# klae01/ddim-audio

Hardware: AMD Instinct MI355X
Metric: DDIM denoising steps/sec (U-Net fwd/s), 1000-step sample, spectrogram batch (higher is better)
Workload: dtype bf16; 1 GPU; BASELINE configs[1]: batch 8/GPU x [2,1024,256] spectrograms, audio.yml U-Net (47.2M params, hash-filled weights; FNet GEMM operands bf16), generalized_steps eta=0 over the 1000-step schedule, one hipGraph per step (inside the forward two batch shards on two streams, fork mask 0x1003f); global_batch=8, t_size=1024, parallelism=batch-sharded x1, no collective in the loop

## Files before the change

### ddim_audio_amd/csrc/api.cpp

```cpp
#include "../../include/ddimx.h"

#include <stdarg.h>
#include <math.h>
#include <stdio.h>
#include <stdlib.h>
#include <string.h>

#include <functional>
#include <string>
#include <vector>

#include "conv_mfma.h"
#include "kernels.h"
#include "train_kernels.h"
#include "wgrad_mfma.h"
#include "conv_pipe.h"

namespace ddimx {
struct Knobs {
    int fnet_dense, conv_pipe, pipe_tpw, bwd_stats_fused, gn_dbg, conv_wreg, conv_wps, conv_var, wgrad_split, wgrad_side, wgrad_hold;
    Knobs() {
        auto geti = [](const char* name, int dflt) { const char* e = getenv(name); return e ? atoi(e) : dflt; };
        conv_var = geti("DDIMX_CONV_VAR", -1);
        conv_wps = geti("DDIMX_CONV_WPS", 0);
// ... 315 lines not shown

static size_t conv_stats_floats(int dtype, int mode, int cin, int cout, int B, int Hv, int Wv) {
    size_t mx = 0;
    for (int var = 0; var < 8; ++var) {
        ConvGeom g;
        if (conv_geometry(dtype, mode, cin, cout, var, &g) != hipSuccess) continue;
        const size_t n = (size_t)B * cdiv(Wv, g.tw) * cdiv(Hv, g.th) * g.classes * g.nout * 2;
        if (n > mx) mx = n;
    }
    if (mode == CONV3 && cin == cout && dtype == DT_BF16) {
        WregGeom wg;
        if (wreg_geometry(CONV3, cin, cout, &wg) == hipSuccess) {
            const size_t n = (size_t)B * cdiv(Wv, wg.tw) * cdiv(Hv, wg.th) * cout * 2;
            if (n > mx) mx = n;
        }
        PipeGeom pg;
        if (pipe_geometry(cin, &pg) == hipSuccess) {
            const size_t n = (size_t)B * cdiv(Wv, pg.tw) * cdiv(Hv, pg.th) * kGnSlab;
            if (n > mx) mx = n;
        }
    }
    if (mode != CONV3 && dtype == DT_BF16) {
        WregGeom wg;
        const int nout = mode == UP4 ? 2 * cout : cout, ncls = mode == UP4 ? 2 : 1;
        if (wreg_geometry(mode, cin, nout, &wg) == hipSuccess) {
            const size_t n = (size_t)B * cdiv(Wv, wg.tw) * cdiv(Hv, wg.th) * ncls * nout * 2;
            if (n > mx) mx = n;
        }
    }
    return mx;
}

static void carve(const ddimx_ctx* c, char* base, int B, int T, Ws* w) {
    const ddimx_config& f = c->cfg;
    const int L = c->L;
    const size_t es = esz(c->dtype);
    Carver cv{base, 0};
    w->temb_h1 = (float*)cv.take((size_t)B * 512 * 4);
    w->temb_h2 = (float*)cv.take((size_t)B * 512 * 4);
    w->temb = (float*)cv.take((size_t)B * c->E * 4);
    const size_t lvl0 = (size_t)B * T * f.f_size * f.ch[0] * es;
    w->A = cv.take(lvl0);
    w->xd.resize(L); w->xu.resize(L);
    size_t stats_f = (size_t)B * conv_in_nparts(T, f.f_size) * (f.ch[0] * 2 > kGnSlab ? f.ch[0] * 2 : kGnSlab);
    size_t hmax = 0;
    int cmax = 0;
    for (int l = 0; l < L; ++l) {
        const int H = T >> l, W = f.f_size >> l, C = f.ch[l];
        const size_t bytes = (size_t)B * H * W * C * es;
        w->xd[l] = cv.take(bytes);
        w->xu[l] = cv.take(bytes);
        if (bytes > hmax) hmax = bytes;
        if (C > cmax) cmax = C;
        size_t s = conv_stats_floats(c->dtype, CONV3, C, C, B, H, W);
        if (s > stats_f) stats_f = s;
        s = (size_t)B * resid_nparts(c->dtype, H * W, C) * (C * 2 > kGnSlab ? C * 2 : kGnSlab);
        if (s > stats_f) stats_f = s;
        if (l > 0) {
            s = conv_stats_floats(c->dtype, DOWN4, f.ch[l - 1], C, B, H, W);
            if (s > stats_f) stats_f = s;
            s = conv_stats_floats(c->dtype, UP4, C, f.ch[l - 1], B, H, W);
            if (s > stats_f) stats_f = s;
        }
    }
    w->h1 = cv.take(hmax);
    w->h2 = cv.take(hmax);
    w->stats_per_sample = stats_f / B;
    w->h_per_sample = hmax / B;
    w->cmax = cmax;
    w->stats = (float*)cv.take(stats_f * 4);
    w->stats2 = (float*)cv.take(stats_f * 4);
    w->scale = (float*)cv.take((size_t)B * cmax * 4);
    w->shift = (float*)cv.take((size_t)B * cmax * 4);
    const int S = T >> (L - 1);
    const size_t M = (size_t)B * S;
    const int hid = f.fnet_hidden, inter = f.fnet_inter;
    w->ln0 = (float*)cv.take((size_t)B * (S > 32 ? S : 32) * c->width * 4);
    w->X = (float*)cv.take(M * hid * 4);
    w->Ut = (float*)cv.take((size_t)B * 2 * hid * S * 4);
    w->Z = (float*)cv.take(M * hid * 4);
    w->Y = (float*)cv.take(M * hid * 4);
    w->Hb = (float*)cv.take(M * inter * 4);
    w->O = (float*)cv.take(M * c->width * 4);
    w->pz = (float*)cv.take((size_t)B * (hid / 16) * 64 * 4);
    w->pv = (float*)cv.take((size_t)B * (hid / 32) * 64 * 4);
    w->zc = (float*)cv.take((size_t)B * 32 * hid * 4);
    w->hc = (float*)cv.take((size_t)B * 32 * inter * 4);
    w->vc = (float*)cv.take((size_t)B * 32 * hid * 4);
    {
        const int bf = c->fnet_bf16;
        const int shp[6][5] = {{(int)M, hid, c->width, 1, bf}, {2 * hid, S, hid, B, 0}, {S, hid, S, B, 0},
                               {(int)M, inter, hid, 1, bf}, {(int)M, hid, inter, 1, bf}, {(int)M, c->width, hid, 1, bf}};
        size_t mx = 0;
        for (auto& q : shp) {
            const size_t n = (size_t)kMaxSplitK * q[3] * q[0] * q[1];
            if (n > mx) mx = n;
        }
        w->gpart_per_sample = mx / B;
        w->gpart = (float*)cv.take(mx * 4);
    }
    w->total = cv.off;
}

struct ConvCall {
    int dtype, mode, cin, cout;
    const void* in; const void* w; const float* bias; const float* chan_add; int chan_add_stride;
    const float* in_scale; const float* in_shift; int xf; int act;
    const void* skip; void* out; float* stats;
    int B, Hin, Win;
    unsigned long long* stamps = nullptr;
    bool batch_plan = false;
    const void* aux = nullptr; const float* aux_scale = nullptr; const float* aux_shift = nullptr; int bwd_mode = 0;
    GnIn gn = {};
    bool groups = false;
    const void* wf = nullptr;
    int kernel_pref = 0;
};

static thread_local bool g_batch_plan = false;
struct BatchPlanScope {
    BatchPlanScope() { g_batch_plan = true; }
    ~BatchPlanScope() { g_batch_plan = false; }
};
struct ConvPlan { ConvGeom g; int var, Hv, Wv, tiles_x, tiles_y, tiles_per_wg, wgs_per_sample; bool wreg, pipe; };
static bool pipe_eligible(const ConvCall& q, PipeGeom* pg) {
    if (q.kernel_pref == 1 || !((knobs().conv_pipe >> (q.cin == 32 ? 0 : 1)) & 1 || q.kernel_pref == 2)) return false;
    if (!q.wf || q.dtype != DT_BF16 || q.mode != CONV3 || q.cin != q.cout || q.act != 1 || q.aux || q.bwd_mode || q.skip || q.batch_plan || g_batch_plan)
        return false;
    if (q.xf != XF_AFFINE && q.xf != XF_AFFINE_SILU) return false;
    if (q.stats && !q.groups) return false;
    if (pipe_geometry(q.cin, pg) != hipSuccess) return false;
    return q.Hin % pg->th == 0 && q.Win % pg->tw == 0;
}
static bool wreg_eligible(const ConvCall& q, WregGeom* wg) {
    if (!knobs().conv_wreg || !q.wf || q.dtype != DT_BF16 || q.act > 1 || q.aux || q.bwd_mode || q.batch_plan || g_batch_plan) return false;
    if (q.skip && q.mode != UP4) return false;
    if (q.xf != XF_NONE && q.xf != XF_AFFINE && q.xf != XF_AFFINE_SILU) return false;
    if (wreg_geometry(q.mode, q.cin, q.mode == UP4 ? 2 * q.cout : q.cout, wg) != hipSuccess) return false;
    const int sxy = q.mode == DOWN4 ? 2 : 1;
    return q.Hin % (wg->th * sxy) == 0 && q.Win % (wg->tw * sxy) == 0;
}
static int conv_plan(const ConvCall& q, ConvPlan* p) {
    ConvGeom& g = p->g;
    p->wreg = false;
    p->pipe = false;
    PipeGeom pgm;
    if (pipe_eligible(q, &pgm)) {
        p->pipe = true;
        p->Hv = q.Hin; p->Wv = q.Win; p->var = 0;
        g.th = pgm.th; g.tw = pgm.tw; g.nb = g.nout = q.cout; g.classes = 1; g.lds_bytes = pgm.lds_bytes; g.nthreads = pgm.nthreads;
        p->tiles_x = q.Win / pgm.tw;
        p->tiles_y = q.Hin / pgm.th;
        const int tiles_s = p->tiles_x * p->tiles_y;
        int tpw = 8;
        if (const int v = knobs().pipe_tpw; v > 0) tpw = q.cin == 32 ? (v & 0xff) : ((v >> 8) ? (v >> 8) : tpw);
        if (tpw > tiles_s) tpw = tiles_s;
        p->tiles_per_wg = tpw;
        p->wgs_per_sample = cdiv(tiles_s, tpw);
        return 0;
    }
    if (q.kernel_pref == 2) return fail("conv %d->%d %dx%d xf=%d act=%d: not eligible for the software-pipelined kernel", q.cin, q.cout, q.Hin, q.Win, q.xf, q.act);
    WregGeom wgm;
    if (wreg_eligible(q, &wgm)) {
        p->wreg = true;
        const int sxy = q.mode == DOWN4 ? 2 : 1;
        p->Hv = q.Hin / sxy; p->Wv = q.Win / sxy; p->var = 0;
        g.th = wgm.th; g.tw = wgm.tw; g.nout = q.mode == UP4 ? 2 * q.cout : q.cout; g.nb = g.nout / wgm.nsplit; g.classes = q.mode == UP4 ? 2 : 1;
        g.lds_bytes = wgm.lds_bytes; g.nthreads = wgm.nthreads;
        p->tiles_x = p->Wv / wgm.tw;
        p->tiles_y = p->Hv / wgm.th;
        const int tiles_s = p->tiles_x * p->tiles_y;
        int wps = tiles_s < 128 ? tiles_s : 128;
        if (tiles_s / 4 > wps) wps = tiles_s / 4;
        if (const int v = knobs().conv_wps; v > 0) wps = v < tiles_s ? v : tiles_s;
        if (q.mode == CONV3 && q.cin == 96 && tiles_s >= 4 && wps > tiles_s / 2) wps = tiles_s / 2;
        if (q.mode != CONV3 && tiles_s >= 64 && cdiv(tiles_s, wps) < 2) wps = tiles_s / 2;
        p->tiles_per_wg = cdiv(tiles_s, wps);
        p->wgs_per_sample = cdiv(tiles_s, p->tiles_per_wg);
        return 0;
    }
    if (q.mode == DOWN4 && ((q.Hin | q.Win) & 1)) return fail("downsample needs even H, W (got %d x %d)", q.Hin, q.Win);
    p->Hv = q.mode == DOWN4 ? q.Hin / 2 : q.Hin;
    p->Wv = q.mode == DOWN4 ? q.Win / 2 : q.Win;
    p->var = conv_pick_variant(q.dtype, q.mode, q.cin, q.cout, (q.batch_plan || g_batch_plan) ? q.B : 0, p->Hv, p->Wv);
    if (conv_geometry(q.dtype, q.mode, q.cin, q.cout, p->var, &g) != hipSuccess)
        return fail("conv %d->%d mode %d dtype %d: no kernel", q.cin, q.cout, q.mode, q.dtype);
    p->tiles_x = cdiv(p->Wv, g.tw);
    p->tiles_y = cdiv(p->Hv, g.th);
    const int tiles_s = p->tiles_x * p->tiles_y;
    int wps = tiles_s < 128 ? tiles_s : 128;
    if (tiles_s / 4 > wps) wps = tiles_s / 4;
    if (q.cin >= 64 && tiles_s >= 512 && wps < 256) wps = 256;
    if (q.mode != CONV3 && tiles_s == 128) wps = 64;
    if (const int v = knobs().conv_wps; v > 0) wps = v < tiles_s ? v : tiles_s;
    p->tiles_per_wg = cdiv(tiles_s, wps);
    p->wgs_per_sample = cdiv(tiles_s, p->tiles_per_wg);
    return 0;
}
constexpr int kNumCUs = 256;
constexpr int kGnFuseConvRounds = 3, kGnFuseResidRounds = 2;
static int conv_rounds(const ConvPlan& p, int B) {
    const long long wgs = (long long)p.wgs_per_sample * B * (p.g.nout / p.g.nb) * p.g.classes;
    int per_cu = (160 * 1024) / p.g.lds_bytes;
    if (per_cu < 1) per_cu = 1;
    if (per_cu > 2048 / p.g.nthreads) per_cu = 2048 / p.g.nthreads;
    return (int)((wgs + (long long)kNumCUs * per_cu - 1) / ((long long)kNumCUs * per_cu));
}
static int run_conv(const ConvCall& q, hipStream_t s, int* nparts, int* Cs) {
    ConvPlan pl;
    CHK(conv_plan(q, &pl));
    const ConvGeom& g = pl.g;
    if (pl.wreg || pl.pipe) {
        WregArgs f;
        memset(&f, 0, sizeof(f));
        f.in = q.in; f.wf = q.wf; f.skip = q.skip; f.bias = q.bias; f.chan_add = q.chan_add; f.chan_add_stride = q.chan_add_stride;
        f.in_scale = q.in_scale; f.in_shift = q.in_shift; f.gn = q.gn; f.out = q.out; f.stats = q.stats;
        f.stats_groups_c = q.groups ? q.cout : 0; f.xf = q.xf; f.act = q.act; f.stamps = q.stamps;
#ifdef DDIMX_STAMP
        { static const int dbg = getenv("DDIMX_PIPE_DBG") ? atoi(getenv("DDIMX_PIPE_DBG")) : 0; f.dbg = dbg; }
#endif
        if (q.gn.stats && q.gn.np > kGnFuseMaxParts) return fail("conv: %d statistics partials per sample cannot be finished in-kernel", q.gn.np);
        if (q.xf != XF_NONE && !q.gn.stats && (!q.in_scale || !q.in_shift)) return fail("conv: affine input without scale / shift");
        f.B = q.B; f.H = q.Hin; f.W = q.Win;
        f.tiles_x = pl.tiles_x; f.tiles_y = pl.tiles_y; f.tiles_per_wg = pl.tiles_per_wg; f.wgs_per_sample = pl.wgs_per_sample;
        if (nparts) *nparts = f.wgs_per_sample * g.classes * (q.groups ? g.nout / g.nb : 1);
        if (Cs) *Cs = g.nout;
        if (pl.pipe) HIPCHK(pipe_launch(q.cin, q.xf, f, s));
        else HIPCHK(wreg_launch(q.mode, q.cin, g.nout, f, s));
        return 0;
    }
    ConvArgs a;
    memset(&a, 0, sizeof(a));
    a.in = q.in; a.w = q.w; a.bias = q.bias; a.chan_add = q.chan_add; a.chan_add_stride = q.chan_add_stride;
    a.in_scale = q.in_scale; a.in_shift = q.in_shift; a.xf = q.xf; a.act = q.act;
    a.skip = q.skip; a.out = q.out; a.stats = q.stats;
    a.gn = q.gn;
    a.aux = q.aux; a.aux_scale = q.aux_scale; a.aux_shift = q.aux_shift; a.bwd_mode = q.bwd_mode;
    a.stats_groups_c = q.groups ? q.cout : 0;
    if (q.gn.stats && q.gn.np > kGnFuseMaxParts) return fail("conv: %d statistics partials per sample cannot be finished in-kernel", q.gn.np);
    if (q.groups && q.cout % kGroups) return fail("conv: group-format statistics need cout %% 8 == 0");
    a.B = q.B; a.Hin = q.Hin; a.Win = q.Win;
    a.stamps = q.stamps;
    a.Hv = pl.Hv; a.Wv = pl.Wv;
    a.tiles_x = pl.tiles_x; a.tiles_y = pl.tiles_y;
    a.tiles_per_wg = pl.tiles_per_wg; a.wgs_per_sample = pl.wgs_per_sample;
    const int var = pl.var;
    if (nparts) *nparts = a.wgs_per_sample * g.classes * (q.groups ? g.nout / g.nb : 1);
    if (Cs) *Cs = g.nout;
    HIPCHK(conv_launch(q.dtype, q.mode, q.cin, q.cout, var, a, s));
    return 0;
}

struct RBPtrs {
    const float *g0, *b0, *g1, *b1, *g2, *bias1;
    const void *w0, *w1;
    const void *w0f = nullptr, *w1f = nullptr;
};

struct RBTape {
    void *u1, *u2;
    float* small;
    float* sc(int i, int B, int C) const { return small + (size_t)(2 * i) * B * C; }
    float* sh(int i, int B, int C) const { return small + (size_t)(2 * i + 1) * B * C; }
    float* mr(int i, int B, int C) const { return small + (size_t)6 * B * C + (size_t)i * B * kGroups * 2; }
};
static inline size_t rb_tape_small_floats(int B, int C) { return (size_t)6 * B * C + (size_t)3 * B * kGroups * 2; }

static int run_resblock(int dtype, int C, const void* x, void* y, const float* temb, int temb_stride, const RBPtrs& p,
                        void* h1, void* h2, float* stats, float* scale, float* shift, int x_nparts, int x_Cs,
                        bool want_stats, int* y_nparts, int B, int H, int W, hipStream_t s, const RBTape* tape = nullptr,
                        float* stats2 = nullptr) {
    const double cnt = (double)H * W * (C / kGroups);
    const float eps = 1e-6f;
    int np = 0, cs = 0;
    if (stats2) {
        if (tape) return fail("run_resblock: the launch-free GroupNorm path keeps no tape");
        auto gn_of = [&](const float* st, int n, const float* gamma, const float* beta, GnIn* g, bool* fused, int which, int rounds,
                         int max_rounds, int nthreads) -> int {
            *g = GnIn{st, gamma, beta, 1.0 / cnt, eps, n};
            *fused = n <= kGnFuseMaxParts && rounds <= max_rounds && !(knobs().gn_dbg & which);
            if (!*fused) HIPCHK(gn_finalize_groups_launch(*g, C, scale, shift, B, nthreads, s));
            return 0;
        };
        GnIn g; bool fu;
        ConvCall k1 = {dtype, CONV3, C, C, x, p.w0, nullptr, temb, temb_stride, scale, shift, XF_AFFINE_SILU, 1, nullptr, h1, stats2, B, H, W};
        k1.groups = true;
        k1.wf = p.w0f;
        ConvPlan pl;
        CHK(conv_plan(k1, &pl));
        CHK(gn_of(stats, x_nparts, p.g0, p.b0, &g, &fu, 2, conv_rounds(pl, B), kGnFuseConvRounds, pl.g.nthreads));
        if (fu) k1.gn = g;
        CHK(run_conv(k1, s, &np, &cs));
        ConvCall k2 = {dtype, CONV3, C, C, h1, p.w1, p.bias1, nullptr, 0, scale, shift, XF_AFFINE, 1, nullptr, h2, stats, B, H, W};
        k2.groups = true;
        k2.wf = p.w1f;
        CHK(conv_plan(k2, &pl));
        CHK(gn_of(stats2, np, p.g1, p.b1, &g, &fu, 2, conv_rounds(pl, B), kGnFuseConvRounds, pl.g.nthreads));
        if (fu) k2.gn = g;
        CHK(run_conv(k2, s, &np, &cs));
        const int rparts = resid_nparts(dtype, H * W, C);
        const int rrounds = (int)(((long long)rparts * B + kNumCUs * 8 - 1) / (kNumCUs * 8));
        CHK(gn_of(stats, np, p.g2, nullptr, &g, &fu, 1, rrounds, kGnFuseResidRounds, resid_threads(dtype, C)));
        HIPCHK(resid_launch(dtype, x, h2, 0, scale, shift, y, want_stats ? stats2 : nullptr, B, H * W, C, s, fu ? &g : nullptr, 1));
        if (y_nparts) *y_nparts = rparts;
        return 0;
    }
    float *sc0 = scale, *sh0 = shift, *sc1 = scale, *sh1 = shift, *sc2 = scale, *sh2 = shift;
// ... 1745 lines not shown
```

### ddim_audio_amd/csrc/conv_inst_bf16_pipe.hip

```cpp
#include "conv_pipe.h"

namespace ddimx {

#define DDIMX_PIPE(X)  \
    X(32, 8, 4, 2)     \
    X(64, 8, 2, 1)

hipError_t pipe_geometry(int c, PipeGeom* g) {
#define DDIMX_G(C_, TH_, WM_, MW_)                                                                        \
    if (c == C_) {                                                                                        \
        typedef PipeCfg<C_, TH_, WM_, XF_AFFINE, MW_> F;                                                  \
        g->th = F::TH; g->tw = F::TW; g->lds_bytes = F::LDS_BYTES; g->nthreads = F::NTHREADS;             \
        return hipSuccess;                                                                                \
    }
    DDIMX_PIPE(DDIMX_G)
    return hipErrorInvalidValue;
}
hipError_t pipe_launch(int c, int xf, const WregArgs& a, hipStream_t stream) {
#ifdef DDIMX_STAMP
#define DDIMX_LD(C_, TH_, WM_, MW_)                                                                      \
    if (c == C_ && a.dbg == 1) return xf == XF_AFFINE ? launch_pipe_cfg<PipeCfg<C_, TH_, WM_, XF_AFFINE, MW_, 1>>(a, stream) : launch_pipe_cfg<PipeCfg<C_, TH_, WM_, XF_AFFINE_SILU, MW_, 1>>(a, stream); \
    if (c == C_ && a.dbg == 2) return xf == XF_AFFINE ? launch_pipe_cfg<PipeCfg<C_, TH_, WM_, XF_AFFINE, MW_, 2>>(a, stream) : launch_pipe_cfg<PipeCfg<C_, TH_, WM_, XF_AFFINE_SILU, MW_, 2>>(a, stream); \
    if (c == C_ && a.dbg == 4) return xf == XF_AFFINE ? launch_pipe_cfg<PipeCfg<C_, TH_, WM_, XF_AFFINE, MW_, 4>>(a, stream) : launch_pipe_cfg<PipeCfg<C_, TH_, WM_, XF_AFFINE_SILU, MW_, 4>>(a, stream); \
    if (c == C_ && a.dbg == 6) return xf == XF_AFFINE ? launch_pipe_cfg<PipeCfg<C_, TH_, WM_, XF_AFFINE, MW_, 6>>(a, stream) : launch_pipe_cfg<PipeCfg<C_, TH_, WM_, XF_AFFINE_SILU, MW_, 6>>(a, stream); \
    if (c == C_ && a.dbg == 7) return xf == XF_AFFINE ? launch_pipe_cfg<PipeCfg<C_, TH_, WM_, XF_AFFINE, MW_, 7>>(a, stream) : launch_pipe_cfg<PipeCfg<C_, TH_, WM_, XF_AFFINE_SILU, MW_, 7>>(a, stream);
    DDIMX_PIPE(DDIMX_LD)
#endif
#define DDIMX_L(C_, TH_, WM_, MW_)                                                                        \
    if (c == C_ && xf == XF_AFFINE) return launch_pipe_cfg<PipeCfg<C_, TH_, WM_, XF_AFFINE, MW_>>(a, stream); \
    if (c == C_ && xf == XF_AFFINE_SILU) return launch_pipe_cfg<PipeCfg<C_, TH_, WM_, XF_AFFINE_SILU, MW_>>(a, stream);
    DDIMX_PIPE(DDIMX_L)
    return hipErrorInvalidValue;
}

}
```

### ddim_audio_amd/csrc/conv_pipe.h

```cpp
#pragma once
#include "conv_wreg.h"

namespace ddimx {

template <int I, int N, class Fn>
__device__ __forceinline__ void static_for(Fn&& f) {
    if constexpr (I < N) {
        f(std::integral_constant<int, I>());
        static_for<I + 1, N>(f);
    }
}

template <int C_, int TH_, int WM_, int XF_, int MINW_ = 1, int DBG_ = 0>
struct PipeCfg {
    static constexpr int C = C_, TH = TH_, TW = 32, WM = WM_, XF = XF_, MINW = MINW_;
    static constexpr int DBG = DBG_;
    static constexpr int WN = C / 32;
    static constexpr int NBLK = C / 32;
    static constexpr int NWAVES = WM * WN, NTHREADS = 64 * NWAVES;
    static constexpr int MT = TH / WM;
    static constexpr int KG = C / 16, NSTEP = 9 * KG;
    static constexpr int NS_TILE = MT * NSTEP;
    static constexpr int IH = TH + 2, IW = TW + 2, NPIX = IH * IW;
    static constexpr int PSTRIDE = C * 2 + 16, ROWSTRIDE = IW * PSTRIDE, HALO_BYTES = IH * ROWSTRIDE;
    static constexpr int LPP = C / 8;
    static constexpr int PPP = NTHREADS / LPP;
    static constexpr int HPT = (NPIX + PPP - 1) / PPP;
    static constexpr int NXE = HPT * 8;
    static constexpr int TR_STRIDE = 80, TR_BYTES = 32 * TR_STRIDE;
    static constexpr int DUMP_BYTES = NTHREADS * 16;
    static constexpr int GN_BYTES = NWAVES * kGroups * 2 * 4;
    static constexpr int OFF_TR = 2 * HALO_BYTES, OFF_DUMP = OFF_TR + NWAVES * TR_BYTES, OFF_GN = OFF_DUMP + DUMP_BYTES;
    static constexpr int LDS_BYTES = OFF_GN + GN_BYTES + 256;
#ifndef DDIMX_PIPE_PD
#define DDIMX_PIPE_PD 2
#endif
    static constexpr int PD = DDIMX_PIPE_PD, NBQ = PD + 1;
    static constexpr int NXU = 4 * HPT, XPB = (NXU + MT - 1) / MT;
    static constexpr int E0 = 2, EP = (NSTEP - 6) / (XPB > 8 ? XPB : 8) > 0 ? (NSTEP - 6) / (XPB > 8 ? XPB : 8) : 1;
    static constexpr int ER = E0 + 8 * EP + 2, ES = ER + 3;
    static constexpr int xstep(int u) { return (u / XPB) * NSTEP + E0 + (u % XPB) * EP; }
    static_assert(C == 32 || C == 64, "widths whose weight fragments fit the register file next to everything else");
    static_assert(TH % WM == 0 && MT % 2 == 0, "blocks per wave must be even (two alternating accumulators across tiles)");
    static_assert(NTHREADS % LPP == 0 && NTHREADS <= 1024, "thread map");
    static_assert(HPT <= 16, "validity masks are 16 bits");
    static_assert(HALO_BYTES + 16 <= 65536, "LDS immediates");
    static_assert(LDS_BYTES <= 160 * 1024, "LDS budget");
    static_assert(ER < ES && ES < NSTEP && E0 + XPB * EP < NSTEP, "filler schedule");
};

template <class F>
__global__ void __launch_bounds__(F::NTHREADS, F::MINW) conv3_pipe_kernel(const WregArgs a) {
    constexpr int C = F::C, XF = F::XF, HPT = F::HPT, NSTEP = F::NSTEP, MT = F::MT;
    constexpr float kNegLog2e = -1.4426950408889634f;
    extern __shared__ __attribute__((aligned(16))) char smem[];
    char* const halo = smem;
    char* const trb = smem + F::OFF_TR;
    char* const dump = smem + F::OFF_DUMP;
    float* const gnscr = (float*)(smem + F::OFF_GN);

    DDIMX_STAMP_ENTRY
    const int tid = threadIdx.x, lane = tid & 63;
    const int wave = __builtin_amdgcn_readfirstlane(tid >> 6);
    const int wm = wave % F::WM, wn = wave / F::WM;
    const int l31 = lane & 31, h = lane >> 5;

    int lwg;
    {
        const int nwg = gridDim.x, x8 = blockIdx.x & 7, i8 = blockIdx.x >> 3;
        const int q = nwg >> 3, r = nwg & 7;
        lwg = (x8 < r ? x8 * (q + 1) : r * (q + 1) + (x8 - r) * q) + i8;
    }
    const int wg = lwg % a.wgs_per_sample;
    const int bs = lwg / a.wgs_per_sample;
    const int ntile_s = a.tiles_x * a.tiles_y;
    const int t_begin = wg * a.tiles_per_wg;
    const int t_end = (t_begin + a.tiles_per_wg < ntile_s) ? t_begin + a.tiles_per_wg : ntile_s;
    const int W_ = a.W;

    uint4 wfr[NSTEP];
    {
        const __amdgpu_buffer_rsrc_t w_rsrc = make_rsrc(a.wf, (unsigned)(9 * C * C * 2));
        const unsigned wlane = (unsigned)((wn * 64 + lane) * 16);
#pragma unroll
        for (int s = 0; s < NSTEP; ++s) {
            const u32x4_t v = __builtin_amdgcn_raw_buffer_load_b128(w_rsrc, wlane, s * (F::NBLK * 1024), 0);
            wfr[s] = make_uint4(v[0], v[1], v[2], v[3]);
        }
    }
    f32x16_t addvec;
    {
        const float* pb = a.bias ? a.bias + wn * 32 + h * 4 : (const float*)a.wf;
        const float* pc = a.chan_add ? a.chan_add + (size_t)bs * a.chan_add_stride + wn * 32 + h * 4 : (const float*)a.wf;
#pragma unroll
        for (int q = 0; q < 4; ++q) {
            const float4 vb = *(const float4*)(pb + (a.bias ? q * 8 : 0));
            const float4 vc = *(const float4*)(pc + (a.chan_add ? q * 8 : 0));
            addvec[q * 4 + 0] = (a.bias ? vb.x : 0.f) + (a.chan_add ? vc.x : 0.f);
            addvec[q * 4 + 1] = (a.bias ? vb.y : 0.f) + (a.chan_add ? vc.y : 0.f);
            addvec[q * 4 + 2] = (a.bias ? vb.z : 0.f) + (a.chan_add ? vc.z : 0.f);
            addvec[q * 4 + 3] = (a.bias ? vb.w : 0.f) + (a.chan_add ? vc.w : 0.f);
        }
    }

    const int hc = tid % F::LPP, hslot = tid / F::LPP;
    unsigned hrel[HPT];
    int hlds[HPT];
    unsigned m_tb = 0, m_lr = 0;
#pragma unroll
    for (int k = 0; k < HPT; ++k) {
        const int pix = k * F::PPP + hslot;
        const bool in = pix < F::NPIX;
        const int iy = pix / F::IW, ix = pix % F::IW;
        hrel[k] = in ? (unsigned)(((iy * W_ + ix) * C + hc * 8) * 2) : 0x80000000u;
        hlds[k] = in ? iy * F::ROWSTRIDE + ix * F::PSTRIDE + hc * 16 : 0;
        if (in && iy == 0) m_tb |= 1u << k;
        if (in && iy == F::IH - 1) m_tb |= 0x10000u << k;
        if (in && ix == 0) m_lr |= 1u << k;
        if (in && ix == F::IW - 1) m_lr |= 0x10000u << k;
    }
    const bool last_in = (HPT - 1) * F::PPP + hslot < F::NPIX;
    char* const my_dump = dump + tid * 16;
    const unsigned in_bytes = (unsigned)((size_t)a.H * W_ * C * 2);
    const char* const in_ptr = (const char*)a.in + (size_t)bs * in_bytes;
    const __amdgpu_buffer_rsrc_t in_rsrc = make_rsrc(in_ptr, in_bytes);
    const __amdgpu_buffer_rsrc_t null_rsrc = make_rsrc(in_ptr, 0u);
    const unsigned out_bytes = in_bytes;
    char* const out_ptr = (char*)a.out + (size_t)bs * out_bytes;
    const __amdgpu_buffer_rsrc_t out_rsrc = make_rsrc(out_ptr, out_bytes);
    const __amdgpu_buffer_rsrc_t out_null = make_rsrc(out_ptr, 0u);

    auto halo_base = [&](int ty, int tx) __attribute__((always_inline)) -> unsigned {
        return (unsigned)(((ty * F::TH - 1) * W_ + tx * F::TW - 1) * (C * 2));
    };
    auto halo_inval = [&](int ty, int tx) __attribute__((always_inline)) -> unsigned {
        const unsigned sel_tb = (ty == 0 ? 0xFFFFu : 0u) | (ty == a.tiles_y - 1 ? 0xFFFF0000u : 0u);
        const unsigned sel_lr = (tx == 0 ? 0xFFFFu : 0u) | (tx == a.tiles_x - 1 ? 0xFFFF0000u : 0u);
        const unsigned x = (m_tb & sel_tb) | (m_lr & sel_lr);
        return (x | (x >> 16)) & 0xFFFFu;
    };

    float sc[8], sh[8];
    {
        const bool gn_fused = a.gn.stats != nullptr;
        GnInLoads gn_ld;
        if (gn_fused) gn_in_issue(a.gn, bs, tid, F::NTHREADS, gn_ld);
        const float* psc = gn_fused ? a.gn.gamma + hc * 8 : a.in_scale + (size_t)bs * C + hc * 8;
        const float* psh = gn_fused ? (a.gn.beta ? a.gn.beta : a.gn.gamma) + hc * 8 : a.in_shift + (size_t)bs * C + hc * 8;
#pragma unroll
        for (int j = 0; j < 8; j += 4) {
            const float4 u = *(const float4*)(psc + j), v = *(const float4*)(psh + j);
            sc[j] = u.x; sc[j + 1] = u.y; sc[j + 2] = u.z; sc[j + 3] = u.w;
            sh[j] = v.x; sh[j + 1] = v.y; sh[j + 2] = v.z; sh[j + 3] = v.w;
        }
        if (gn_fused) {
            gn_in_reduce(a.gn, bs, tid, F::NTHREADS, gn_ld, gnscr);
            __syncthreads();
            float bet[8], fs[8], fh[8];
#pragma unroll
            for (int j = 0; j < 8; ++j) bet[j] = a.gn.beta ? sh[j] : 0.f;
            gn_in_fold<8>(a.gn, gnscr, F::NWAVES, C, hc * 8, sc, bet, fs, fh);
#pragma unroll
            for (int j = 0; j < 8; ++j) { sc[j] = fs[j]; sh[j] = fh[j]; }
        }
    }

    uint4 hreg[HPT];
    unsigned xw[4];
    auto word_of = [&](auto k_, auto w_) __attribute__((always_inline)) -> unsigned {
        constexpr int k = decltype(k_)::value, w = decltype(w_)::value;
        return w == 0 ? hreg[k].x : (w == 1 ? hreg[k].y : (w == 2 ? hreg[k].z : hreg[k].w));
    };
    float xy[2][2], xe[2][2];
    auto xf_a = [&](auto k_, auto p_) __attribute__((always_inline)) {
        constexpr int p = decltype(p_)::value;
        const unsigned w0 = word_of(k_, p_);
        const float x0 = __uint_as_float(w0 << 16), x1 = __uint_as_float(w0 & 0xffff0000u);
        const float y0 = fmaf(x0, sc[2 * p], sh[2 * p]), y1 = fmaf(x1, sc[2 * p + 1], sh[2 * p + 1]);
        xy[p & 1][0] = y0; xy[p & 1][1] = y1;
        if constexpr (XF == XF_AFFINE_SILU) {
            xe[p & 1][0] = __builtin_amdgcn_exp2f(y0 * kNegLog2e);
            xe[p & 1][1] = __builtin_amdgcn_exp2f(y1 * kNegLog2e);
        }
    };
    auto xf_b = [&](auto k_, auto p_) __attribute__((always_inline)) {
        constexpr int p = decltype(p_)::value;
        float y0 = xy[p & 1][0], y1 = xy[p & 1][1];
        if constexpr (XF == XF_AFFINE_SILU) {
            y0 *= __builtin_amdgcn_rcpf(xe[p & 1][0] + 1.0f);
            y1 *= __builtin_amdgcn_rcpf(xe[p & 1][1] + 1.0f);
        }
        xw[p] = Piece<__bf16>::pk(y0, y1);
    };
    auto xf_finish = [&](auto k_, char* hdst, unsigned inval, __amdgpu_buffer_rsrc_t nrsrc, unsigned nbase) __attribute__((always_inline)) {
        constexpr int k = decltype(k_)::value;
        const bool bad = (inval >> k) & 1u;
        uint4 v;
        v.x = bad ? 0u : xw[0];
        v.y = bad ? 0u : xw[1];
        v.z = bad ? 0u : xw[2];
        v.w = bad ? 0u : xw[3];
        char* dst = hdst + hlds[k];
        if constexpr (k == HPT - 1) dst = last_in ? dst : my_dump;
        *(uint4*)dst = v;
        hreg[k] = buf_load16(nrsrc, nbase + hrel[k]);
    };

    float st_s[4], st_q[4];
#pragma unroll
    for (int q = 0; q < 4; ++q) { st_s[q] = 0.f; st_q[q] = 0.f; }
    char* const tr_w = trb + wave * F::TR_BYTES + l31 * F::TR_STRIDE + h * 8;
    const char* const tr_r = trb + wave * F::TR_BYTES + (lane >> 2) * F::TR_STRIDE + (lane & 3) * 16;
    const unsigned st_lane = (unsigned)((lane >> 2) * (C * 2) + wn * 64 + (lane & 3) * 16);
    uint4 trv[2];
    unsigned ow[2];
    float ev[2][2], ee[2][2];
    auto epi_a = [&](const f32x16_t& acc, auto e_) __attribute__((always_inline)) {
        constexpr int e = decltype(e_)::value, q = e / 2, i2 = e % 2;
        const float v0 = acc[q * 4 + 2 * i2], v1 = acc[q * 4 + 2 * i2 + 1];
        ev[i2][0] = v0; ev[i2][1] = v1;
        ee[i2][0] = __builtin_amdgcn_exp2f(v0 * kNegLog2e);
        ee[i2][1] = __builtin_amdgcn_exp2f(v1 * kNegLog2e);
    };
    auto epi_b = [&](auto e_) __attribute__((always_inline)) {
        constexpr int e = decltype(e_)::value, q = e / 2, i2 = e % 2;
        const float v0 = ev[i2][0] * __builtin_amdgcn_rcpf(ee[i2][0] + 1.0f);
        const float v1 = ev[i2][1] * __builtin_amdgcn_rcpf(ee[i2][1] + 1.0f);
        st_s[q] += v0; st_q[q] = fmaf(v0, v0, st_q[q]);
        st_s[q] += v1; st_q[q] = fmaf(v1, v1, st_q[q]);
        ow[i2] = Piece<__bf16>::pk(v0, v1);
        if constexpr (i2 == 1) *(uint2*)(tr_w + q * 16) = make_uint2(ow[0], ow[1]);
    };
    auto epi_readback = [&]() __attribute__((always_inline)) {
        trv[0] = *(const uint4*)(tr_r);
        trv[1] = *(const uint4*)(tr_r + 16 * F::TR_STRIDE);
    };
    auto epi_store = [&](__amdgpu_buffer_rsrc_t orsrc, unsigned rowbase) __attribute__((always_inline)) {
        const u32x4_t t0 = {trv[0].x, trv[0].y, trv[0].z, trv[0].w}, t1 = {trv[1].x, trv[1].y, trv[1].z, trv[1].w};
        const unsigned rb = __builtin_amdgcn_readfirstlane(rowbase);
        __builtin_amdgcn_raw_buffer_store_b128(t0, orsrc, st_lane, rb, 0);
        __builtin_amdgcn_raw_buffer_store_b128(t1, orsrc, st_lane + 16 * C * 2, rb, 0);
    };

    int ty = t_begin / a.tiles_x, tx = t_begin % a.tiles_x;
    int ty2 = ty, tx2 = tx;
    auto advance = [&](int& y, int& x) __attribute__((always_inline)) { if (++x == a.tiles_x) { x = 0; ++y; } };
    {
        const unsigned b0 = halo_base(ty2, tx2);
#pragma unroll
        for (int k = 0; k < HPT; ++k) hreg[k] = buf_load16(in_rsrc, b0 + hrel[k]);
    }
    unsigned inval_a = halo_inval(ty2, tx2);
    advance(ty2, tx2);
    {
        const bool has1 = t_begin + 1 < t_end;
        const __amdgpu_buffer_rsrc_t r1 = has1 ? in_rsrc : null_rsrc;
        const unsigned b1 = halo_base(ty2, tx2);
        const unsigned inval_b = halo_inval(ty2, tx2);
        static_for<0, HPT>([&](auto k_) {
            static_for<0, 4>([&](auto p_) { xf_a(k_, p_); xf_b(k_, p_); });
            xf_finish(k_, halo, inval_a, r1, b1);
        });
        inval_a = inval_b;
        advance(ty2, tx2);
    }
    f32x16_t acc0, acc1;
#pragma unroll
    for (int r = 0; r < 16; ++r) { acc0[r] = 0.f; acc1[r] = 0.f; }
    unsigned prev_rowbase = 0;
    __amdgpu_buffer_rsrc_t prev_rsrc = out_null;
    const int lanebase = wm * MT * F::ROWSTRIDE + l31 * F::PSTRIDE + h * 16;
    asm volatile("s_waitcnt lgkmcnt(0)" ::: "memory");
    __builtin_amdgcn_s_barrier();
    asm volatile("" ::: "memory");
    DDIMX_STAMP_DECL

    auto body = [&](auto xfn_, int cur, int t) __attribute__((always_inline)) {
        constexpr bool XFN = decltype(xfn_)::value;
        if constexpr (XFN) asm volatile("; tile body, a next tile exists" : "+v"(acc1));
        else asm volatile("; tile body, last tile of the workgroup" : "+v"(acc1));
        const char* const hsrc = halo + cur * F::HALO_BYTES + lanebase;
        char* const hdst = halo + (cur ^ 1) * F::HALO_BYTES;
        const bool has2 = t + 2 < t_end;
        const __amdgpu_buffer_rsrc_t r2 = has2 ? in_rsrc : null_rsrc;
        const unsigned b2 = halo_base(ty2, tx2);
        const unsigned inval_b = halo_inval(ty2, tx2);
        const unsigned rowbase = (unsigned)(((ty * F::TH + wm * MT) * W_ + tx * F::TW) * (C * 2));
        uint4 bq[F::NBQ];
        auto lds_b = [&](auto g_) __attribute__((always_inline)) -> uint4 {
            constexpr int G = decltype(g_)::value, m = G / NSTEP, s = G % NSTEP, tap = s / F::KG, kg = s % F::KG;
            constexpr int off = (m + tap / 3) * F::ROWSTRIDE + (tap % 3) * F::PSTRIDE + kg * 32;
            return *(const uint4*)(hsrc + off);
        };
        static_for<0, F::PD>([&](auto g_) { bq[decltype(g_)::value % F::NBQ] = lds_b(g_); });
        __builtin_amdgcn_sched_barrier(0);
        static_for<0, F::NS_TILE>([&](auto g_) {
            constexpr int G = decltype(g_)::value, m = G / NSTEP, s = G % NSTEP;
            if constexpr (G + F::PD < F::NS_TILE) bq[(G + F::PD) % F::NBQ] = lds_b(std::integral_constant<int, G + F::PD>());
            {
                f32x16_t& acc = (m & 1) ? acc1 : acc0;
                const bf16x8_t av = __builtin_bit_cast(bf16x8_t, wfr[s]), bv = __builtin_bit_cast(bf16x8_t, bq[G % F::NBQ]);
                if constexpr (F::DBG & 1) { if constexpr (s == 0) acc = addvec; asm volatile("" :: "v"(av), "v"(bv)); }
                else if constexpr (s == 0) acc = __builtin_amdgcn_mfma_f32_32x32x16_bf16(av, bv, addvec, 0, 0, 0);
                else acc = __builtin_amdgcn_mfma_f32_32x32x16_bf16(av, bv, acc, 0, 0, 0);
            }
            if constexpr (XFN && !(F::DBG & 2)) {
                static_for<0, F::NXU>([&](auto u_) {
                    constexpr int u = decltype(u_)::value;
                    if constexpr (F::xstep(u) + F::EP == G) {
                        xf_b(std::integral_constant<int, u / 4>(), std::integral_constant<int, u % 4>());
                        if constexpr (u % 4 == 3) xf_finish(std::integral_constant<int, u / 4>(), hdst, inval_a, r2, b2);
                    }
                });
                static_for<0, F::NXU>([&](auto u_) {
                    constexpr int u = decltype(u_)::value;
                    if constexpr (F::xstep(u) == G) xf_a(std::integral_constant<int, u / 4>(), std::integral_constant<int, u % 4>());
                });
            }
            if constexpr (!(F::DBG & 4)) {
                const f32x16_t& pacc = (m & 1) ? acc0 : acc1;
                static_for<0, 8>([&](auto e_) {
                    if constexpr (s == F::E0 + (decltype(e_)::value + 1) * F::EP) epi_b(e_);
                });
                static_for<0, 8>([&](auto e_) {
                    if constexpr (s == F::E0 + decltype(e_)::value * F::EP) epi_a(pacc, e_);
                });
                if constexpr (s == F::ER) epi_readback();
                if constexpr (s == F::ES) {
                    if constexpr (m == 0) epi_store(prev_rsrc, prev_rowbase);
                    else epi_store(out_rsrc, rowbase + (unsigned)((m - 1) * W_ * (C * 2)));
                }
            }
            __builtin_amdgcn_sched_barrier(0);
        });
        inval_a = inval_b;
        prev_rowbase = rowbase + (unsigned)((MT - 1) * W_ * (C * 2));
        prev_rsrc = out_rsrc;
    };

#pragma unroll 1
    for (int t = t_begin; t < t_end; ++t) {
        const int cur = (t - t_begin) & 1;
        if (t + 1 < t_end) body(std::true_type(), cur, t);
        else body(std::false_type(), cur, t);
        advance(ty, tx);
        advance(ty2, tx2);
        DDIMX_STAMP_AT(0);
        asm volatile("s_waitcnt lgkmcnt(0)" ::: "memory");
        __builtin_amdgcn_s_barrier();
        asm volatile("" ::: "memory");
        DDIMX_STAMP_AT(1);
    }
    static_for<0, 8>([&](auto e_) { epi_a(acc1, e_); epi_b(e_); });
    epi_readback();
    epi_store(prev_rsrc, prev_rowbase);
    DDIMX_STAMP_AT(2);

    if (a.stats) {
        float* const red = (float*)smem;
#pragma unroll
        for (int o = 1; o < 32; o <<= 1) {
#pragma unroll
            for (int q = 0; q < 4; ++q) {
                st_s[q] += __shfl_xor(st_s[q], o, 64);
                st_q[q] += __shfl_xor(st_q[q], o, 64);
            }
        }
        if (l31 == 0) {
#pragma unroll
            for (int q = 0; q < 4; ++q) *(float2*)(red + ((wave * 2 + h) * 4 + q) * 2) = make_float2(st_s[q], st_q[q]);
        }
        __syncthreads();
        if (tid < kGnSlab) {
            float tot = 0.f;
            if (tid < 2 * kGroups) {
                const int g = tid >> 1, sq = tid & 1;
                constexpr int GS = C / kGroups;
#pragma unroll
                for (int w = 0; w < F::NWAVES; ++w)
#pragma unroll
                    for (int hh = 0; hh < 2; ++hh)
#pragma unroll
                        for (int q = 0; q < 4; ++q) {
                            const int ch = (w / F::WM) * 32 + q * 8 + hh * 4;
                            const float v = red[((w * 2 + hh) * 4 + q) * 2 + sq];
                            tot += (ch / GS == g) ? v : 0.f;
                        }
            }
            a.stats[((size_t)bs * a.wgs_per_sample + wg) * kGnSlab + tid] = tot;
        }
    }
    DDIMX_STAMP_AT(3);
    DDIMX_STAMP_FLUSH();
}

template <class F>
hipError_t launch_pipe_cfg(const WregArgs& a, hipStream_t stream) {
    static bool attr_done = false;
    if (!attr_done) {
        hipError_t e = hipFuncSetAttribute((const void*)conv3_pipe_kernel<F>, hipFuncAttributeMaxDynamicSharedMemorySize, F::LDS_BYTES);
        if (e != hipSuccess) return e;
        attr_done = true;
    }
    hipLaunchKernelGGL(conv3_pipe_kernel<F>, dim3(a.wgs_per_sample * a.B), dim3(F::NTHREADS), F::LDS_BYTES, stream, a);
    return hipGetLastError();
}

struct PipeGeom { int th, tw, lds_bytes, nthreads; };
hipError_t pipe_geometry(int c, PipeGeom* g);
hipError_t pipe_launch(int c, int xf, const WregArgs& a, hipStream_t stream);

}
```

Before: 2348 sample-fwd/s.

## Split K across wave pairs in the pipelined 64-channel conv kernel

For 64-channel convolutions the pipelined kernel now splits the reduction over input-channel groups between two waves. Each wave holds half the weight fragments and the partial sums are exchanged through LDS slots that alternate by tile parity. The tile shrinks to 2 rows with one M wave, and the default tiles per workgroup for C=64 goes to 16. This is meant to cut per-wave register pressure and raise occupancy and MFMA parallelism, at the cost of extra LDS traffic for the partials and more complex epilogue ordering that could be fragile.

```diff
diff --git a/ddim_audio_amd/csrc/api.cpp b/ddim_audio_amd/csrc/api.cpp
--- a/ddim_audio_amd/csrc/api.cpp
+++ b/ddim_audio_amd/csrc/api.cpp
@@ -491,7 +491,7 @@
         p->tiles_x = q.Win / pgm.tw;
         p->tiles_y = q.Hin / pgm.th;
         const int tiles_s = p->tiles_x * p->tiles_y;
-        int tpw = 8;
+        int tpw = q.cin == 32 ? 8 : 16;
         if (const int v = knobs().pipe_tpw; v > 0) tpw = q.cin == 32 ? (v & 0xff) : ((v >> 8) ? (v >> 8) : tpw);
         if (tpw > tiles_s) tpw = tiles_s;
         p->tiles_per_wg = tpw;
diff --git a/ddim_audio_amd/csrc/conv_inst_bf16_pipe.hip b/ddim_audio_amd/csrc/conv_inst_bf16_pipe.hip
--- a/ddim_audio_amd/csrc/conv_inst_bf16_pipe.hip
+++ b/ddim_audio_amd/csrc/conv_inst_bf16_pipe.hip
@@ -2,14 +2,14 @@
 
 namespace ddimx {
 
-#define DDIMX_PIPE(X)  \
-    X(32, 8, 4, 2)     \
-    X(64, 8, 2, 1)
+#define DDIMX_PIPE(X)     \
+    X(32, 8, 4, 2, 1)     \
+    X(64, 2, 1, 2, 2)
 
 hipError_t pipe_geometry(int c, PipeGeom* g) {
-#define DDIMX_G(C_, TH_, WM_, MW_)                                                                        \
+#define DDIMX_G(C_, TH_, WM_, MW_, KS_)                                                                      \
     if (c == C_) {                                                                                        \
-        typedef PipeCfg<C_, TH_, WM_, XF_AFFINE, MW_> F;                                                  \
+        typedef PipeCfg<C_, TH_, WM_, XF_AFFINE, MW_, 0, KS_> F;                                        \
         g->th = F::TH; g->tw = F::TW; g->lds_bytes = F::LDS_BYTES; g->nthreads = F::NTHREADS;             \
         return hipSuccess;                                                                                \
     }
@@ -18,17 +18,17 @@
 }
 hipError_t pipe_launch(int c, int xf, const WregArgs& a, hipStream_t stream) {
 #ifdef DDIMX_STAMP
-#define DDIMX_LD(C_, TH_, WM_, MW_)                                                                      \
-    if (c == C_ && a.dbg == 1) return xf == XF_AFFINE ? launch_pipe_cfg<PipeCfg<C_, TH_, WM_, XF_AFFINE, MW_, 1>>(a, stream) : launch_pipe_cfg<PipeCfg<C_, TH_, WM_, XF_AFFINE_SILU, MW_, 1>>(a, stream); \
-    if (c == C_ && a.dbg == 2) return xf == XF_AFFINE ? launch_pipe_cfg<PipeCfg<C_, TH_, WM_, XF_AFFINE, MW_, 2>>(a, stream) : launch_pipe_cfg<PipeCfg<C_, TH_, WM_, XF_AFFINE_SILU, MW_, 2>>(a, stream); \
-    if (c == C_ && a.dbg == 4) return xf == XF_AFFINE ? launch_pipe_cfg<PipeCfg<C_, TH_, WM_, XF_AFFINE, MW_, 4>>(a, stream) : launch_pipe_cfg<PipeCfg<C_, TH_, WM_, XF_AFFINE_SILU, MW_, 4>>(a, stream); \
-    if (c == C_ && a.dbg == 6) return xf == XF_AFFINE ? launch_pipe_cfg<PipeCfg<C_, TH_, WM_, XF_AFFINE, MW_, 6>>(a, stream) : launch_pipe_cfg<PipeCfg<C_, TH_, WM_, XF_AFFINE_SILU, MW_, 6>>(a, stream); \
-    if (c == C_ && a.dbg == 7) return xf == XF_AFFINE ? launch_pipe_cfg<PipeCfg<C_, TH_, WM_, XF_AFFINE, MW_, 7>>(a, stream) : launch_pipe_cfg<PipeCfg<C_, TH_, WM_, XF_AFFINE_SILU, MW_, 7>>(a, stream);
+#define DDIMX_LD(C_, TH_, WM_, MW_, KS_)                                                                     \
+    if (c == C_ && a.dbg == 1) return xf == XF_AFFINE ? launch_pipe_cfg<PipeCfg<C_, TH_, WM_, XF_AFFINE, MW_, 1, KS_>>(a, stream) : launch_pipe_cfg<PipeCfg<C_, TH_, WM_, XF_AFFINE_SILU, MW_, 1, KS_>>(a, stream); \
+    if (c == C_ && a.dbg == 2) return xf == XF_AFFINE ? launch_pipe_cfg<PipeCfg<C_, TH_, WM_, XF_AFFINE, MW_, 2, KS_>>(a, stream) : launch_pipe_cfg<PipeCfg<C_, TH_, WM_, XF_AFFINE_SILU, MW_, 2, KS_>>(a, stream); \
+    if (c == C_ && a.dbg == 4) return xf == XF_AFFINE ? launch_pipe_cfg<PipeCfg<C_, TH_, WM_, XF_AFFINE, MW_, 4, KS_>>(a, stream) : launch_pipe_cfg<PipeCfg<C_, TH_, WM_, XF_AFFINE_SILU, MW_, 4, KS_>>(a, stream); \
+    if (c == C_ && a.dbg == 6) return xf == XF_AFFINE ? launch_pipe_cfg<PipeCfg<C_, TH_, WM_, XF_AFFINE, MW_, 6, KS_>>(a, stream) : launch_pipe_cfg<PipeCfg<C_, TH_, WM_, XF_AFFINE_SILU, MW_, 6, KS_>>(a, stream); \
+    if (c == C_ && a.dbg == 7) return xf == XF_AFFINE ? launch_pipe_cfg<PipeCfg<C_, TH_, WM_, XF_AFFINE, MW_, 7, KS_>>(a, stream) : launch_pipe_cfg<PipeCfg<C_, TH_, WM_, XF_AFFINE_SILU, MW_, 7, KS_>>(a, stream);
     DDIMX_PIPE(DDIMX_LD)
 #endif
-#define DDIMX_L(C_, TH_, WM_, MW_)                                                                        \
-    if (c == C_ && xf == XF_AFFINE) return launch_pipe_cfg<PipeCfg<C_, TH_, WM_, XF_AFFINE, MW_>>(a, stream); \
-    if (c == C_ && xf == XF_AFFINE_SILU) return launch_pipe_cfg<PipeCfg<C_, TH_, WM_, XF_AFFINE_SILU, MW_>>(a, stream);
+#define DDIMX_L(C_, TH_, WM_, MW_, KS_)                                                                      \
+    if (c == C_ && xf == XF_AFFINE) return launch_pipe_cfg<PipeCfg<C_, TH_, WM_, XF_AFFINE, MW_, 0, KS_>>(a, stream); \
+    if (c == C_ && xf == XF_AFFINE_SILU) return launch_pipe_cfg<PipeCfg<C_, TH_, WM_, XF_AFFINE_SILU, MW_, 0, KS_>>(a, stream);
     DDIMX_PIPE(DDIMX_L)
     return hipErrorInvalidValue;
 }
diff --git a/ddim_audio_amd/csrc/conv_pipe.h b/ddim_audio_amd/csrc/conv_pipe.h
--- a/ddim_audio_amd/csrc/conv_pipe.h
+++ b/ddim_audio_amd/csrc/conv_pipe.h
@@ -11,16 +11,18 @@
     }
 }
 
-template <int C_, int TH_, int WM_, int XF_, int MINW_ = 1, int DBG_ = 0>
+template <int C_, int TH_, int WM_, int XF_, int MINW_ = 1, int DBG_ = 0, int KS_ = 1>
 struct PipeCfg {
     static constexpr int C = C_, TH = TH_, TW = 32, WM = WM_, XF = XF_, MINW = MINW_;
     static constexpr int DBG = DBG_;
+    static constexpr int KS = KS_;
     static constexpr int WN = C / 32;
     static constexpr int NBLK = C / 32;
-    static constexpr int NWAVES = WM * WN, NTHREADS = 64 * NWAVES;
+    static constexpr int NWAVES = WM * WN * KS, NTHREADS = 64 * NWAVES;
     static constexpr int MT = TH / WM;
     static constexpr int KG = C / 16, NSTEP = 9 * KG;
-    static constexpr int NS_TILE = MT * NSTEP;
+    static constexpr int KGS = KG / KS, NSB = NSTEP / KS;
+    static constexpr int NS_TILE = MT * NSB;
     static constexpr int IH = TH + 2, IW = TW + 2, NPIX = IH * IW;
     static constexpr int PSTRIDE = C * 2 + 16, ROWSTRIDE = IW * PSTRIDE, HALO_BYTES = IH * ROWSTRIDE;
     static constexpr int LPP = C / 8;
@@ -28,30 +30,33 @@
     static constexpr int HPT = (NPIX + PPP - 1) / PPP;
     static constexpr int NXE = HPT * 8;
     static constexpr int TR_STRIDE = 80, TR_BYTES = 32 * TR_STRIDE;
+    static constexpr int PART_BYTES = 16 * 64 * 4, TRR_BYTES = KS == 1 ? NWAVES * TR_BYTES : 2 * NWAVES * PART_BYTES;
     static constexpr int DUMP_BYTES = NTHREADS * 16;
     static constexpr int GN_BYTES = NWAVES * kGroups * 2 * 4;
-    static constexpr int OFF_TR = 2 * HALO_BYTES, OFF_DUMP = OFF_TR + NWAVES * TR_BYTES, OFF_GN = OFF_DUMP + DUMP_BYTES;
+    static constexpr int OFF_TR = 2 * HALO_BYTES, OFF_DUMP = OFF_TR + TRR_BYTES, OFF_GN = OFF_DUMP + DUMP_BYTES;
     static constexpr int LDS_BYTES = OFF_GN + GN_BYTES + 256;
 #ifndef DDIMX_PIPE_PD
 #define DDIMX_PIPE_PD 2
 #endif
     static constexpr int PD = DDIMX_PIPE_PD, NBQ = PD + 1;
     static constexpr int NXU = 4 * HPT, XPB = (NXU + MT - 1) / MT;
-    static constexpr int E0 = 2, EP = (NSTEP - 6) / (XPB > 8 ? XPB : 8) > 0 ? (NSTEP - 6) / (XPB > 8 ? XPB : 8) : 1;
+    static constexpr int E0 = 2, EP = (NSB - 6) / (XPB > 8 ? XPB : 8) > 0 ? (NSB - 6) / (XPB > 8 ? XPB : 8) : 1;
     static constexpr int ER = E0 + 8 * EP + 2, ES = ER + 3;
-    static constexpr int xstep(int u) { return (u / XPB) * NSTEP + E0 + (u % XPB) * EP; }
+    static constexpr int PW = 2;
+    static constexpr int xstep(int u) { return (u / XPB) * NSB + E0 + (u % XPB) * EP; }
     static_assert(C == 32 || C == 64, "widths whose weight fragments fit the register file next to everything else");
+    static_assert(KS == 1 || (KS == 2 && WM == 1 && MT == 2 && KG % 2 == 0), "K split: one wave per (cout block, K half), two blocks per tile");
     static_assert(TH % WM == 0 && MT % 2 == 0, "blocks per wave must be even (two alternating accumulators across tiles)");
     static_assert(NTHREADS % LPP == 0 && NTHREADS <= 1024, "thread map");
     static_assert(HPT <= 16, "validity masks are 16 bits");
     static_assert(HALO_BYTES + 16 <= 65536, "LDS immediates");
     static_assert(LDS_BYTES <= 160 * 1024, "LDS budget");
-    static_assert(ER < ES && ES < NSTEP && E0 + XPB * EP < NSTEP, "filler schedule");
+    static_assert(ER < ES && ES < NSB && E0 + XPB * EP < NSB && PW + 4 < NSB, "filler schedule");
 };
 
 template <class F>
 __global__ void __launch_bounds__(F::NTHREADS, F::MINW) conv3_pipe_kernel(const WregArgs a) {
-    constexpr int C = F::C, XF = F::XF, HPT = F::HPT, NSTEP = F::NSTEP, MT = F::MT;
+    constexpr int C = F::C, XF = F::XF, HPT = F::HPT, NSB = F::NSB, MT = F::MT, KS = F::KS;
     constexpr float kNegLog2e = -1.4426950408889634f;
     extern __shared__ __attribute__((aligned(16))) char smem[];
     char* const halo = smem;
@@ -62,7 +67,8 @@
     DDIMX_STAMP_ENTRY
     const int tid = threadIdx.x, lane = tid & 63;
     const int wave = __builtin_amdgcn_readfirstlane(tid >> 6);
-    const int wm = wave % F::WM, wn = wave / F::WM;
+    const int wm = wave % F::WM, wn = (wave / F::WM) % F::WN, ks = wave / (F::WM * F::WN);
+    const int partner = wave ^ (KS == 2 ? F::WM * F::WN : 0);
     const int l31 = lane & 31, h = lane >> 5;
 
     int lwg;
@@ -78,13 +84,13 @@
     const int t_end = (t_begin + a.tiles_per_wg < ntile_s) ? t_begin + a.tiles_per_wg : ntile_s;
     const int W_ = a.W;
 
-    uint4 wfr[NSTEP];
+    uint4 wfr[NSB];
     {
         const __amdgpu_buffer_rsrc_t w_rsrc = make_rsrc(a.wf, (unsigned)(9 * C * C * 2));
-        const unsigned wlane = (unsigned)((wn * 64 + lane) * 16);
-#pragma unroll
-        for (int s = 0; s < NSTEP; ++s) {
-            const u32x4_t v = __builtin_amdgcn_raw_buffer_load_b128(w_rsrc, wlane, s * (F::NBLK * 1024), 0);
+        const unsigned wlane = (unsigned)((wn * 64 + lane) * 16 + ks * F::KGS * (F::NBLK * 1024));
+#pragma unroll
+        for (int s = 0; s < NSB; ++s) {
+            const u32x4_t v = __builtin_amdgcn_raw_buffer_load_b128(w_rsrc, wlane, ((s / F::KGS) * F::KG + s % F::KGS) * (F::NBLK * 1024), 0);
             wfr[s] = make_uint4(v[0], v[1], v[2], v[3]);
         }
     }
@@ -209,15 +215,26 @@
     float st_s[4], st_q[4];
 #pragma unroll
     for (int q = 0; q < 4; ++q) { st_s[q] = 0.f; st_q[q] = 0.f; }
-    char* const tr_w = trb + wave * F::TR_BYTES + l31 * F::TR_STRIDE + h * 8;
-    const char* const tr_r = trb + wave * F::TR_BYTES + (lane >> 2) * F::TR_STRIDE + (lane & 3) * 16;
+    const int tr_lw = l31 * F::TR_STRIDE + h * 8, tr_lr = (lane >> 2) * F::TR_STRIDE + (lane & 3) * 16;
+    auto part_slot = [&](int parity, int w) __attribute__((always_inline)) -> char* { return trb + (parity * F::NWAVES + w) * F::PART_BYTES; };
+    char* tr_w = trb + wave * F::TR_BYTES + tr_lw;
+    const char* tr_r = trb + wave * F::TR_BYTES + tr_lr;
     const unsigned st_lane = (unsigned)((lane >> 2) * (C * 2) + wn * 64 + (lane & 3) * 16);
     uint4 trv[2];
     unsigned ow[2];
     float ev[2][2], ee[2][2];
+    float pr[16];
+    auto epi_part = [&](const char* slot) __attribute__((always_inline)) {
+#pragma unroll
+        for (int i = 0; i < 4; ++i) {
+            const float4 v = *(const float4*)(slot + i * 1024 + lane * 16);
+            pr[4 * i] = v.x; pr[4 * i + 1] = v.y; pr[4 * i + 2] = v.z; pr[4 * i + 3] = v.w;
+        }
+    };
     auto epi_a = [&](const f32x16_t& acc, auto e_) __attribute__((always_inline)) {
         constexpr int e = decltype(e_)::value, q = e / 2, i2 = e % 2;
-        const float v0 = acc[q * 4 + 2 * i2], v1 = acc[q * 4 + 2 * i2 + 1];
+        float v0 = acc[q * 4 + 2 * i2], v1 = acc[q * 4 + 2 * i2 + 1];
+        if constexpr (KS == 2) { v0 += pr[q * 4 + 2 * i2]; v1 += pr[q * 4 + 2 * i2 + 1]; }
         ev[i2][0] = v0; ev[i2][1] = v1;
         ee[i2][0] = __builtin_amdgcn_exp2f(v0 * kNegLog2e);
         ee[i2][1] = __builtin_amdgcn_exp2f(v1 * kNegLog2e);
@@ -264,12 +281,16 @@
         inval_a = inval_b;
         advance(ty2, tx2);
     }
-    f32x16_t acc0, acc1;
-#pragma unroll
-    for (int r = 0; r < 16; ++r) { acc0[r] = 0.f; acc1[r] = 0.f; }
+    f32x16_t acc0, acc1, zero16;
+#pragma unroll
+    for (int r = 0; r < 16; ++r) { acc0[r] = 0.f; acc1[r] = 0.f; zero16[r] = 0.f; }
     unsigned prev_rowbase = 0;
     __amdgpu_buffer_rsrc_t prev_rsrc = out_null;
-    const int lanebase = wm * MT * F::ROWSTRIDE + l31 * F::PSTRIDE + h * 16;
+    const int lanebase = wm * MT * F::ROWSTRIDE + l31 * F::PSTRIDE + h * 16 + ks * F::KGS * 32;
+    if constexpr (KS == 2) {
+#pragma unroll
+        for (int i = 0; i < 4; ++i) *(uint4*)(part_slot(1, wave) + i * 1024 + lane * 16) = make_uint4(0u, 0u, 0u, 0u);
+    }
     asm volatile("s_waitcnt lgkmcnt(0)" ::: "memory");
     __builtin_amdgcn_s_barrier();
     asm volatile("" ::: "memory");
@@ -286,22 +307,32 @@
         const unsigned b2 = halo_base(ty2, tx2);
         const unsigned inval_b = halo_inval(ty2, tx2);
         const unsigned rowbase = (unsigned)(((ty * F::TH + wm * MT) * W_ + tx * F::TW) * (C * 2));
+        const int hrow0 = KS == 2 ? (1 - ks) * F::ROWSTRIDE : 0, hrow1 = KS == 2 ? ks * F::ROWSTRIDE : 0;
+        char* const part_w = part_slot(cur, wave);
+        char* const part_r = part_slot(cur ^ 1, partner);
+        if constexpr (KS == 2) {
+            char* const rd = part_r;
+            tr_w = rd + tr_lw;
+            tr_r = rd + tr_lr;
+        }
         uint4 bq[F::NBQ];
         auto lds_b = [&](auto g_) __attribute__((always_inline)) -> uint4 {
-            constexpr int G = decltype(g_)::value, m = G / NSTEP, s = G % NSTEP, tap = s / F::KG, kg = s % F::KG;
-            constexpr int off = (m + tap / 3) * F::ROWSTRIDE + (tap % 3) * F::PSTRIDE + kg * 32;
-            return *(const uint4*)(hsrc + off);
+            constexpr int G = decltype(g_)::value, m = G / NSB, s = G % NSB, tap = s / F::KGS, kg = s % F::KGS;
+            constexpr int off = (KS == 1 ? m : 0) * F::ROWSTRIDE + (tap / 3) * F::ROWSTRIDE + (tap % 3) * F::PSTRIDE + kg * 32;
+            return *(const uint4*)(hsrc + (KS == 1 ? 0 : (m == 0 ? hrow0 : hrow1)) + off);
         };
         static_for<0, F::PD>([&](auto g_) { bq[decltype(g_)::value % F::NBQ] = lds_b(g_); });
+        if constexpr (KS == 2 && !(F::DBG & 4)) epi_part(part_r);
         __builtin_amdgcn_sched_barrier(0);
         static_for<0, F::NS_TILE>([&](auto g_) {
-            constexpr int G = decltype(g_)::value, m = G / NSTEP, s = G % NSTEP;
+            constexpr int G = decltype(g_)::value, m = G / NSB, s = G % NSB;
             if constexpr (G + F::PD < F::NS_TILE) bq[(G + F::PD) % F::NBQ] = lds_b(std::integral_constant<int, G + F::PD>());
             {
                 f32x16_t& acc = (m & 1) ? acc1 : acc0;
                 const bf16x8_t av = __builtin_bit_cast(bf16x8_t, wfr[s]), bv = __builtin_bit_cast(bf16x8_t, bq[G % F::NBQ]);
-                if constexpr (F::DBG & 1) { if constexpr (s == 0) acc = addvec; asm volatile("" :: "v"(av), "v"(bv)); }
-                else if constexpr (s == 0) acc = __builtin_amdgcn_mfma_f32_32x32x16_bf16(av, bv, addvec, 0, 0, 0);
+                const f32x16_t& init = (KS == 2 && m == 0) ? zero16 : addvec;
+                if constexpr (F::DBG & 1) { if constexpr (s == 0) acc = init; asm volatile("" :: "v"(av), "v"(bv)); }
+                else if constexpr (s == 0) acc = __builtin_amdgcn_mfma_f32_32x32x16_bf16(av, bv, init, 0, 0, 0);
                 else acc = __builtin_amdgcn_mfma_f32_32x32x16_bf16(av, bv, acc, 0, 0, 0);
             }
             if constexpr (XFN && !(F::DBG & 2)) {
@@ -317,7 +348,7 @@
                     if constexpr (F::xstep(u) == G) xf_a(std::integral_constant<int, u / 4>(), std::integral_constant<int, u % 4>());
                 });
             }
-            if constexpr (!(F::DBG & 4)) {
+            if constexpr (!(F::DBG & 4) && (KS == 1 || m == 0)) {
                 const f32x16_t& pacc = (m & 1) ? acc0 : acc1;
                 static_for<0, 8>([&](auto e_) {
                     if constexpr (s == F::E0 + (decltype(e_)::value + 1) * F::EP) epi_b(e_);
@@ -331,10 +362,14 @@
                     else epi_store(out_rsrc, rowbase + (unsigned)((m - 1) * W_ * (C * 2)));
                 }
             }
+            if constexpr (KS == 2 && m == 1 && s >= F::PW && s < F::PW + 4) {
+                constexpr int i = s - F::PW;
+                *(float4*)(part_w + i * 1024 + lane * 16) = make_float4(acc0[4 * i], acc0[4 * i + 1], acc0[4 * i + 2], acc0[4 * i + 3]);
+            }
             __builtin_amdgcn_sched_barrier(0);
         });
         inval_a = inval_b;
-        prev_rowbase = rowbase + (unsigned)((MT - 1) * W_ * (C * 2));
+        prev_rowbase = rowbase + (unsigned)((KS == 2 ? ks : MT - 1) * W_ * (C * 2));
         prev_rsrc = out_rsrc;
     };
 
@@ -351,6 +386,12 @@
         asm volatile("" ::: "memory");
         DDIMX_STAMP_AT(1);
     }
+    if constexpr (KS == 2) {
+        char* const rd = part_slot(((t_end - t_begin) & 1) ^ 1, partner);
+        tr_w = rd + tr_lw;
+        tr_r = rd + tr_lr;
+        epi_part(rd);
+    }
     static_for<0, 8>([&](auto e_) { epi_a(acc1, e_); epi_b(e_); });
     epi_readback();
     epi_store(prev_rsrc, prev_rowbase);
@@ -382,7 +423,7 @@
                     for (int hh = 0; hh < 2; ++hh)
 #pragma unroll
                         for (int q = 0; q < 4; ++q) {
-                            const int ch = (w / F::WM) * 32 + q * 8 + hh * 4;
+                            const int ch = ((w / F::WM) % F::WN) * 32 + q * 8 + hh * 4;
                             const float v = red[((w * 2 + hh) * 4 + q) * 2 + sq];
                             tot += (ch / GS == g) ? v : 0.f;
                         }
```

Result: no change. 2348 sample-fwd/s, median of 6 (-0.0%).
